# vimalabs/VIMA

Hardware: NVIDIA H100
Metric: policy steps/sec (batched action decode) (higher is better)
Workload: dtype f16 hi*hi + e4m3 cross terms (2 tensor pass-equivalents), f16 3-term in attention, fp32 accumulate/softmax/LN

## Files before the change

vima_b200/csrc/api.cu:

```cuda
#include <cstdarg>
#include <cstddef>
#include <cstdio>
#include <cstring>
#include <cstdlib>

#include "../../include/vima_b200.h"
#include "gemm_wide.cuh"
#include "kernels.h"

using namespace vima;
static_assert(VIMA_KV_PAGE_TOKENS == KV_PAGE_TOKENS, "page size of the C ABI and of the kernels");

struct vima_ctx {
  int device;
  int sm_count;
  int max_smem_optin;
  long long launches;
  char err[512];
  void* encode_tiled;
  int attn_tc;
  int attn_tail;
  int epi_prefetch;
  int attn_bias_tc;
  int gemm_wide;
};

struct DeviceGuard {
  int prev = -1;
  bool armed = false;
  cudaError_t enter(int dev) {
    cudaError_t e = cudaGetDevice(&prev);
    if (e != cudaSuccess) return e;
    if (prev == dev) return cudaSuccess;
    armed = true;
    return cudaSetDevice(dev);
  }
  ~DeviceGuard() {
    if (armed) cudaSetDevice(prev);
  }
};

static int fail(vima_ctx* c, int code, const char* fmt, ...) {
  if (c) {
    va_list ap;
    va_start(ap, fmt);
    vsnprintf(c->err, sizeof(c->err), fmt, ap);
    va_end(ap);
  }
  return code;
}
static int cuda_fail(vima_ctx* c, cudaError_t e, const char* what) {
  return fail(c, VIMA_E_CUDA, "%s: %s", what, cudaGetErrorString(e));
}
#define CHECK_CTX(c)                  \
  if (!(c)) return VIMA_E_INVALID;    \
  DeviceGuard dev_guard_;             \
  {                                   \
// ... 10 lines not shown
                what, sz, min_size, sizeof(D), VIMA_B200_ABI_VERSION);
  memset(out, 0, sizeof(D));
  memcpy(out, in, sz);
  return VIMA_OK;
}
#define LAUNCHED(c, expr, name)                          \
  {                                                      \
    cudaError_t e_ = (expr);                             \
    if (e_ != cudaSuccess) return cuda_fail((c), e_, name); \
    (c)->launches++;                                     \
    return VIMA_OK;                                      \
  }

extern "C" {

int vima_abi_version(void) { return VIMA_B200_ABI_VERSION; }

int vima_set_option(vima_ctx* c, const char* key, const char* value) {
  if (!c) return VIMA_E_INVALID;
  if (!key || !value) return fail(c, VIMA_E_INVALID, "set_option: null key or value");
  if (!strcmp(key, "attn")) {
    if (!strcmp(value, "tc")) { c->attn_tc = 1; return VIMA_OK; }
    if (!strcmp(value, "mma")) { c->attn_tc = 0; return VIMA_OK; }
  } else if (!strcmp(key, "attn_tail")) {
    if (!strcmp(value, "kernel")) { c->attn_tail = 1; return VIMA_OK; }
    if (!strcmp(value, "off")) { c->attn_tail = 0; return VIMA_OK; }
  } else if (!strcmp(key, "attn_bias")) {
    if (!strcmp(value, "auto")) { c->attn_bias_tc = 0; return VIMA_OK; }
    if (!strcmp(value, "tc")) { c->attn_bias_tc = 1; return VIMA_OK; }
  } else if (!strcmp(key, "epi_prefetch")) {
    if (!strcmp(value, "0") || !strcmp(value, "1")) { c->epi_prefetch = value[0] == '1'; return VIMA_OK; }
  } else if (!strcmp(key, "gemm_wide")) {
    if (!strcmp(value, "0") || !strcmp(value, "1")) { c->gemm_wide = value[0] == '1'; return VIMA_OK; }
  }
  return fail(c, VIMA_E_INVALID, "set_option: unknown option %s=%s", key, value);
}

int vima_create(vima_ctx** out, int device) {
  if (!out) return VIMA_E_INVALID;
  *out = nullptr;
  int n = 0;
  if (cudaGetDeviceCount(&n) != cudaSuccess || device < 0 || device >= n) return VIMA_E_CUDA;
  cudaDeviceProp prop;
  if (cudaGetDeviceProperties(&prop, device) != cudaSuccess) return VIMA_E_CUDA;
  if (prop.major != 9 || prop.minor != 0) return VIMA_E_UNSUPPORTED;
  vima_ctx* c = new vima_ctx();
  memset(c, 0, sizeof(*c));
  c->device = device;
  c->sm_count = prop.multiProcessorCount;
  c->max_smem_optin = (int)prop.sharedMemPerBlockOptin;
  DeviceGuard guard;
  if (guard.enter(device) != cudaSuccess) { delete c; return VIMA_E_CUDA; }
  cudaFree(0);
  cudaDriverEntryPointQueryResult q;
  void* fn = nullptr;
  if (cudaGetDriverEntryPoint("cuTensorMapEncodeTiled", &fn, cudaEnableDefault, &q) != cudaSuccess || fn == nullptr) {
    delete c;
    return VIMA_E_CUDA;
  }
  c->encode_tiled = fn;
  c->attn_tc = 1; c->attn_tail = 1; c->epi_prefetch = 0; c->attn_bias_tc = 0; c->gemm_wide = 1;
  if (const char* e = getenv("VIMA_B200_ATTN")) vima_set_option(c, "attn", e);
  if (const char* e = getenv("VIMA_B200_ATTN_TAIL")) vima_set_option(c, "attn_tail", e);
  if (const char* e = getenv("VIMA_B200_EPI_PREFETCH")) vima_set_option(c, "epi_prefetch", e);
  if (const char* e = getenv("VIMA_B200_ATTN_BIAS")) vima_set_option(c, "attn_bias", e);
  if (const char* e = getenv("VIMA_B200_GEMM_WIDE")) vima_set_option(c, "gemm_wide", e);
  c->err[0] = 0;
  *out = c;
  return VIMA_OK;
}

void vima_destroy(vima_ctx* c) { delete c; }
const char* vima_last_error(vima_ctx* c) { return c ? c->err : "null context"; }
int vima_sm_count(vima_ctx* c) { return c ? c->sm_count : 0; }
int vima_sizeof_gemm_desc(void) { return (int)sizeof(vima_gemm_desc); }
int vima_sizeof_norm_desc(void) { return (int)sizeof(vima_norm_desc); }
int vima_sizeof_attn_desc(void) { return (int)sizeof(vima_attn_desc); }
int vima_sizeof_f32_gemm_group(void) { return (int)sizeof(vima_f32_gemm_group); }
int64_t vima_launch_count(vima_ctx* c) { return c ? c->launches : 0; }

int vima_split_f32(vima_ctx* c, const float* x, int64_t rows, int cols, int ldx, void* hi, void* lo, int ld16, int pad_cols, float scale,
                   int dtype, void* stream) {
  CHECK_CTX(c);
  if (!x || !hi || pad_cols < cols || pad_cols > ld16) return fail(c, VIMA_E_INVALID, "split_f32: bad arguments");
  LAUNCHED(c, launch_split(x, rows, cols, ldx, (unsigned short*)hi, (unsigned short*)lo, ld16, pad_cols, scale, dtype, (cudaStream_t)stream),
           "split_f32");
}

int vima_pack_weight(vima_ctx* c, const float* w, int n, int k, int transposed, int ldw, void* hi, void* lo, int ld16, float scale, int dtype,
                     void* stream) {
  CHECK_CTX(c);
  if (!w || !hi || ld16 < k || (ld16 & 7)) return fail(c, VIMA_E_INVALID, "pack_weight: ld16 must be >= k and a multiple of 8");
  LAUNCHED(c, launch_pack_weight(w, n, k, transposed, ldw, (unsigned short*)hi, (unsigned short*)lo, ld16, scale, dtype, (cudaStream_t)stream),
           "pack_weight");
}

int vima_pack_weight_f8(vima_ctx* c, const float* w, int n, int k, int transposed, int ldw, void* hi8, void* lo8, int ld8, float scale, void* stream) {
  CHECK_CTX(c);
  if (!w || !hi8 || !lo8 || ld8 < k || (ld8 & 15)) return fail(c, VIMA_E_INVALID, "pack_weight_f8: ld8 must be >= k and a multiple of 16");
// ... 11 lines not shown
  const int step = glu ? 64 : 32;
  int best = step, best_pad = 1 << 30;
  for (int bn = step; bn <= GEMM_MAX_BN; bn += step) {
    const int padded = ((N + bn - 1) / bn) * bn;
    if (padded < best_pad || (padded == best_pad && bn > best)) { best = bn; best_pad = padded; }
  }
  return best;
}
int vima_glu_block_n(int n_out) { return choose_block_n(2 * n_out, 1); }
int vima_gemm_stats_parts(int N, int glu, int block_n) {
  const int bn = block_n > 0 ? block_n : choose_block_n(N, glu);
  return 2 * ((N + bn - 1) / bn);
}

int vima_row_stats_finalize(vima_ctx* c, const float* partial, int64_t rows, int parts, int cols, float eps, int rms, float* stats, void* stream) {
  CHECK_CTX(c);
  if (!partial || !stats || rows < 0 || parts <= 0 || cols <= 0 || ((uintptr_t)partial & 7) || ((uintptr_t)stats & 7))
    return fail(c, VIMA_E_INVALID, "row_stats_finalize: bad arguments");
  LAUNCHED(c, launch_row_stats_finalize(partial, rows, parts, cols, eps, rms, stats, (cudaStream_t)stream), "row_stats_finalize");
}

static int make_tmap_f8(vima_ctx* c, CUtensorMap* tm, const void* base, int rows, int cols, int ld, int box_rows) {
  CUresult r = encode_tmap_2d(c->encode_tiled, tm, CU_TENSOR_MAP_DATA_TYPE_UINT8, base, (uint64_t)rows, (uint64_t)cols, (uint64_t)ld, GEMM_BK,
                              (uint32_t)box_rows, CU_TENSOR_MAP_SWIZZLE_64B, CU_TENSOR_MAP_L2_PROMOTION_L2_256B);
  if (r != CUDA_SUCCESS) return fail(c, VIMA_E_CUDA, "cuTensorMapEncodeTiled(fp8) failed (%d): rows %d cols %d ld %d box %d", (int)r, rows, cols, ld, box_rows);
  return VIMA_OK;
}

static int make_tmap(vima_ctx* c, CUtensorMap* tm, const void* base, int dtype, int rows, int cols, int ld, int box_rows) {
  const CUtensorMapDataType dt = dtype == DT_BF16 ? CU_TENSOR_MAP_DATA_TYPE_BFLOAT16 : CU_TENSOR_MAP_DATA_TYPE_FLOAT16;
  CUresult r = encode_tmap_2d(c->encode_tiled, tm, dt, base, (uint64_t)rows, (uint64_t)cols, (uint64_t)ld * 2, GEMM_BK, (uint32_t)box_rows,
                              CU_TENSOR_MAP_SWIZZLE_128B, CU_TENSOR_MAP_L2_PROMOTION_L2_256B);
  if (r != CUDA_SUCCESS) return fail(c, VIMA_E_CUDA, "cuTensorMapEncodeTiled failed (%d): rows %d cols %d ld %d box %d", (int)r, rows, cols, ld, box_rows);
  return VIMA_OK;
}

int vima_gemm(vima_ctx* c, const vima_gemm_desc* d_in, void* stream) {
  CHECK_CTX(c);
  vima_gemm_desc d_local;
  if (int rc_ = load_desc(c, d_in, &d_local, VIMA_GEMM_DESC_V4_SIZE, "gemm")) return rc_;
  const vima_gemm_desc* d = &d_local;
  if (!d->a_hi || !d->b_hi) return fail(c, VIMA_E_INVALID, "gemm: null operand");
  if (d->M <= 0 || d->N <= 0 || d->K <= 0) return fail(c, VIMA_E_INVALID, "gemm: empty problem");
  if ((d->lda & 7) || (d->ldb & 7) || ((uintptr_t)d->a_hi & 15) || ((uintptr_t)d->b_hi & 15))
    return fail(c, VIMA_E_INVALID, "gemm: operands need 16-byte aligned bases and ld %% 8 == 0 (lda %d ldb %d)", d->lda, d->ldb);
  if ((d->a_lo == nullptr) != (d->b_lo == nullptr)) return fail(c, VIMA_E_INVALID, "gemm: a_lo and b_lo must both be set or both be null");
  const bool f8 = d->a_lo8 || d->a_hi8 || d->b_hi8 || d->b_lo8;
  if (f8) {
    if (!(d->a_lo8 && d->a_hi8 && d->b_hi8 && d->b_lo8) || d->a_lo || d->dtype != DT_F16)
      return fail(c, VIMA_E_INVALID, "gemm: f16f8 mode needs all four e4m3 operands, fp16 hi operands and no 16-bit lo operands");
    if ((d->lda8 & 15) || (d->ldb8 & 15) || ((uintptr_t)d->a_lo8 & 15) || ((uintptr_t)d->a_hi8 & 15) || ((uintptr_t)d->b_hi8 & 15) ||
        ((uintptr_t)d->b_lo8 & 15) || d->lda8 < d->K || d->ldb8 < d->K)
      return fail(c, VIMA_E_INVALID, "gemm: e4m3 operands need 16-byte aligned bases and ld %% 16 == 0");
  }
  if ((d->out_lo8 == nullptr) != (d->out_hi8 == nullptr) || (d->out_lo8 && (!d->out_hi || d->dtype != DT_F16 || (d->ld_o8 & 3))))
    return fail(c, VIMA_E_INVALID, "gemm: out_lo8/out_hi8 come together, with an fp16 out_hi, ld_o8 %% 4 == 0");
  if (d->lda < d->K || d->ldb < d->K) return fail(c, VIMA_E_INVALID, "gemm: leading dimension smaller than K");
  int bn = d->block_n > 0 ? d->block_n : choose_block_n(d->N, d->glu);
  if (bn > GEMM_MAX_BN || (bn % (d->glu ? 64 : 32))) return fail(c, VIMA_E_INVALID, "gemm: bad block_n %d (multiple of 32, 64 with GLU, <= %d)", bn, GEMM_MAX_BN);
  if (d->glu && (d->N % bn)) return fail(c, VIMA_E_INVALID, "gemm: GLU needs N %% block_n == 0");
  {
    const int n_out = d->glu ? d->N / 2 : d->N;
    const bool bad = (n_out & 3) || (d->out_f32 && ((d->ld_o32 & 3) || ((uintptr_t)d->out_f32 & 15))) ||
                     (d->out_hi && ((d->ld_o16 & 3) || ((uintptr_t)d->out_hi & 7) || (d->out_lo && ((uintptr_t)d->out_lo & 7)))) ||
                     (d->mul && ((d->ld_mul & 3) || ((uintptr_t)d->mul & 15))) || (d->residual && ((d->ld_res & 3) || ((uintptr_t)d->residual & 15)));
    if (bad) return fail(c, VIMA_E_INVALID, "gemm: epilogue tensors need N %% 4 == 0, ld %% 4 == 0 and 16-byte (fp32) / 8-byte (16-bit) aligned bases");
// ... 22 lines not shown
  l.split = split; l.block_n = bn;
  const bool wide = c->gemm_wide && split == 2 && bn == 128 && d->N % GEMM_WIDE_BN == 0 && gemm_wide_has_epilogue(l) &&
                    gemm_wide_smem_bytes() <= (size_t)c->max_smem_optin;
  const int tile_n = wide ? GEMM_WIDE_BN : bn;
  int rc;
  const int tiles_m_ = (d->M + GEMM_BM - 1) / GEMM_BM, tiles_n_ = (d->N + tile_n - 1) / tile_n;
  if ((rc = make_tmap(c, &p.tm_a_hi, d->a_hi, d->dtype, d->M, d->K, d->lda, GEMM_BM))) return rc;
  if ((rc = make_tmap(c, &p.tm_b_hi, d->b_hi, d->dtype, d->N, d->K, d->ldb, tile_n))) return rc;
  if (split == 1) {
    if ((rc = make_tmap(c, &p.tm_a_lo, d->a_lo, d->dtype, d->M, d->K, d->lda, GEMM_BM))) return rc;
    if ((rc = make_tmap(c, &p.tm_b_lo, d->b_lo, d->dtype, d->N, d->K, d->ldb, bn))) return rc;
  } else if (split == 2) {
    if ((rc = make_tmap_f8(c, &p.tm_a_lo, d->a_lo8, d->M, d->K, d->lda8, GEMM_BM))) return rc;
    if ((rc = make_tmap_f8(c, &p.tm_a_hi8, d->a_hi8, d->M, d->K, d->lda8, GEMM_BM))) return rc;
    if ((rc = make_tmap_f8(c, &p.tm_b_hi8, d->b_hi8, d->N, d->K, d->ldb8, tile_n))) return rc;
    if ((rc = make_tmap_f8(c, &p.tm_b_lo, d->b_lo8, d->N, d->K, d->ldb8, tile_n))) return rc;
  }
  p.M = d->M; p.N = d->N; p.K = d->K;
  p.dtype = d->dtype;
  p.glu = d->glu;
  p.epi_prefetch = c->epi_prefetch;
  p.act = d->act;
  p.acc_scale = d->acc_scale == 0.f ? 1.f : d->acc_scale;
  p.bias = d->bias;
  p.mul = d->mul; p.ld_mul = d->ld_mul;
  p.residual = d->residual; p.ld_res = d->ld_res;
  p.out_f32 = d->out_f32; p.ld_o32 = d->ld_o32;
  p.out_hi = (unsigned short*)d->out_hi; p.out_lo = (unsigned short*)d->out_lo; p.ld_o16 = d->ld_o16;
  p.out_lo8 = (unsigned char*)d->out_lo8; p.out_hi8 = (unsigned char*)d->out_hi8; p.ld_o8 = d->ld_o8;
  p.row_stats = d->row_stats; p.ln_c1 = d->ln_c1; p.ln_cols = d->ln_cols;
  p.res_stats = d->res_stats; p.res_gamma = d->res_gamma; p.res_beta = d->res_beta;
  p.stats_out = d->stats_out; p.stats_parts = d->stats_parts;

  const int tiles = tiles_m_ * tiles_n_;
  const int grid = tiles < c->sm_count ? tiles : c->sm_count;
  if (wide) LAUNCHED(c, launch_gemm_wide(p, l, grid, gemm_wide_smem_bytes(), c->max_smem_optin, (cudaStream_t)stream), "gemm_wide_kernel");
  const size_t stage = (size_t)(GEMM_A_TILE_BYTES + bn * 128) * (split ? 2 : 1);
  const size_t fixed = gemm_smem_bytes(bn, split, 0);
  int n_stages = (int)(((size_t)c->max_smem_optin - fixed) / stage);
  if (n_stages > GEMM_MAX_STAGES) n_stages = GEMM_MAX_STAGES;
  if (n_stages < 2) return fail(c, VIMA_E_UNSUPPORTED, "gemm: not enough shared memory for 2 stages");
  p.n_stages = n_stages;
  const size_t smem = gemm_smem_bytes(bn, split, n_stages);
  auto launch = d->dtype == DT_BF16 ? (split ? launch_gemm_tc<DT_BF16, 1> : launch_gemm_tc<DT_BF16, 0>)
                                    : (split == 2 ? launch_gemm_tc<DT_F16, 2> : split ? launch_gemm_tc<DT_F16, 1> : launch_gemm_tc<DT_F16, 0>);
  LAUNCHED(c, launch(p, l, grid, smem, c->max_smem_optin, (cudaStream_t)stream), "gemm_tc_kernel");
}

int vima_gemm_f32_grouped(vima_ctx* c, const vima_f32_gemm_group* groups_dev, int n_groups, int M, int max_n, int act, void* stream) {
  CHECK_CTX(c);
  static_assert(sizeof(vima_f32_gemm_group) == sizeof(SimtGemmGroup), "group layout");
  if (!groups_dev) return fail(c, VIMA_E_INVALID, "gemm_f32_grouped: null groups");
  LAUNCHED(c, launch_simt_gemm_grouped(reinterpret_cast<const SimtGemmGroup*>(groups_dev), n_groups, M, max_n, act, (cudaStream_t)stream),
           "simt_gemm");
}

int vima_gemm_f32_grouped_host(vima_ctx* c, const vima_f32_gemm_group* groups_host, int n_groups, int M, int max_n, int act, void* stream) {
  CHECK_CTX(c);
  if (!groups_host || n_groups < 0) return fail(c, VIMA_E_INVALID, "gemm_f32_grouped_host: null groups");
  if (M < 0) return fail(c, VIMA_E_INVALID, "gemm_f32_grouped_host: M = %d < 0", M);
  for (int i = 0; i < n_groups; ++i)
    if (groups_host[i].n > max_n)
      return fail(c, VIMA_E_INVALID, "gemm_f32_grouped_host: group %d has n = %d columns, more than max_n = %d", i, groups_host[i].n, max_n);
  cudaError_t e = launch_simt_gemm_grouped_host(reinterpret_cast<const SimtGemmGroup*>(groups_host), n_groups, M, max_n, act, (cudaStream_t)stream);
  if (e != cudaSuccess) return cuda_fail(c, e, "simt_gemm");
  c->launches += (n_groups + SIMT_MAX_HOST_GROUPS - 1) / SIMT_MAX_HOST_GROUPS;
// ... 341 lines not shown
```

vima_b200/csrc/common.cuh:

```cuda
#pragma once
#include <cuda.h>
#include <cuda_bf16.h>
#include <cuda_fp16.h>
#include <cuda_runtime.h>
#include <stdint.h>
#include <stdio.h>

#ifndef VIMA_WAIT_CYCLES
#define VIMA_WAIT_CYCLES (3000000000ll)
#endif

namespace vima {

enum : int { DT_F16 = 0, DT_BF16 = 1 };
enum : int { ACT_NONE = 0, ACT_RELU = 1, ACT_QUICKGELU = 2, ACT_GELU = 3, ACT_GELU_TANH = 4 };

__device__ __forceinline__ uint32_t smem_u32(const void* p) { return (uint32_t)__cvta_generic_to_shared(p); }

template <int DT>
struct Op16;
template <>
struct Op16<DT_F16> {
  using T = __half;
  static __device__ __forceinline__ unsigned short bits(float x) { return __half_as_ushort(__float2half_rn(x)); }
// ... 105 lines not shown
__device__ __forceinline__ void mbar_arrive(uint64_t* bar) {
  asm volatile("mbarrier.arrive.shared::cta.b64 _, [%0];" ::"r"(smem_u32(bar)) : "memory");
}
__device__ __forceinline__ bool mbar_try_wait(uint64_t* bar, uint32_t parity) {
  uint32_t ok;
  asm volatile(
      "{\n\t.reg .pred p;\n\t"
      "mbarrier.try_wait.parity.shared::cta.b64 p, [%1], %2;\n\t"
      "selp.u32 %0, 1, 0, p;\n\t}"
      : "=r"(ok)
      : "r"(smem_u32(bar)), "r"(parity)
      : "memory");
  return ok != 0;
}
__device__ __forceinline__ void mbar_wait(uint64_t* bar, uint32_t parity) {
  if (mbar_try_wait(bar, parity)) return;
  const long long t0 = clock64();
  uint32_t spins = 0;
  while (!mbar_try_wait(bar, parity)) {
    if ((++spins & 1023u) == 0u && clock64() - t0 > VIMA_WAIT_CYCLES) __trap();
  }
}

__device__ __forceinline__ void tma_prefetch_desc(const void* tmap) {
  asm volatile("prefetch.tensormap [%0];" ::"l"(tmap) : "memory");
}
__device__ __forceinline__ void tma_load_2d(void* smem_dst, const void* tmap, uint64_t* bar, int c0, int c1) {
  asm volatile(
      "cp.async.bulk.tensor.2d.shared::cluster.global.mbarrier::complete_tx::bytes [%0], [%1, {%3, %4}], [%2];" ::"r"(
          smem_u32(smem_dst)),
      "l"(tmap), "r"(smem_u32(bar)), "r"(c0), "r"(c1)
      : "memory");
}

__device__ __forceinline__ uint64_t wgmma_desc_sw128(uint32_t smem_addr) {
  return (uint64_t)((smem_addr >> 4) & 0x3FFF) | (1ull << 16) | ((uint64_t)(1024 >> 4) << 32) | (1ull << 62);
}
__device__ __forceinline__ uint64_t wgmma_desc_sw64(uint32_t smem_addr) {
  return (uint64_t)((smem_addr >> 4) & 0x3FFF) | (1ull << 16) | ((uint64_t)(512 >> 4) << 32) | (2ull << 62);
}
__device__ __forceinline__ void wgmma_fence() { asm volatile("wgmma.fence.sync.aligned;" ::: "memory"); }
__device__ __forceinline__ void wgmma_commit() { asm volatile("wgmma.commit_group.sync.aligned;" ::: "memory"); }
template <int N>
__device__ __forceinline__ void wgmma_wait() { asm volatile("wgmma.wait_group.sync.aligned %0;" ::"n"(N) : "memory"); }
template <int N>
__device__ __forceinline__ void wgmma_fence_acc(float (&d)[N]) {
#pragma unroll
  for (int i = 0; i < N; ++i) asm volatile("" : "+f"(d[i])::"memory");
}

#define VIMA_ACC8(d, o)                                                                                                  \
  "+f"(d[(o) + 0]), "+f"(d[(o) + 1]), "+f"(d[(o) + 2]), "+f"(d[(o) + 3]), "+f"(d[(o) + 4]), "+f"(d[(o) + 5]), "+f"(d[(o) + 6]), \
      "+f"(d[(o) + 7])
#define VIMA_ACC16(d) VIMA_ACC8(d, 0), VIMA_ACC8(d, 8)
#define VIMA_ACC32(d) VIMA_ACC16(d), VIMA_ACC8(d, 16), VIMA_ACC8(d, 24)
#define VIMA_ACC48(d) VIMA_ACC32(d), VIMA_ACC8(d, 32), VIMA_ACC8(d, 40)
#define VIMA_ACC64(d) VIMA_ACC48(d), VIMA_ACC8(d, 48), VIMA_ACC8(d, 56)
#define VIMA_R16 "{%0, %1, %2, %3, %4, %5, %6, %7, %8, %9, %10, %11, %12, %13, %14, %15}"
#define VIMA_R32 \
  "{%0, %1, %2, %3, %4, %5, %6, %7, %8, %9, %10, %11, %12, %13, %14, %15, %16, %17, %18, %19, %20, %21, %22, %23, %24, %25, %26, %27, %28, %29, %30, %31}"
#define VIMA_R48 \
  "{%0, %1, %2, %3, %4, %5, %6, %7, %8, %9, %10, %11, %12, %13, %14, %15, %16, %17, %18, %19, %20, %21, %22, %23, %24, %25, %26, %27, %28, %29, %30, %31, %32, %33, %34, %35, %36, %37, %38, %39, %40, %41, %42, %43, %44, %45, %46, %47}"
#define VIMA_R64 \
  "{%0, %1, %2, %3, %4, %5, %6, %7, %8, %9, %10, %11, %12, %13, %14, %15, %16, %17, %18, %19, %20, %21, %22, %23, %24, %25, %26, %27, %28, %29, %30, %31, %32, %33, %34, %35, %36, %37, %38, %39, %40, %41, %42, %43, %44, %45, %46, %47, %48, %49, %50, %51, %52, %53, %54, %55, %56, %57, %58, %59, %60, %61, %62, %63}"

#define VIMA_WGMMA_K16(N, R, ACC, IA, IB, IP)                                                                                      \
// ... 81 lines not shown
```

vima_b200/csrc/gemm_tc.cuh:

```cuda
#pragma once
#include "common.cuh"

namespace vima {

constexpr int GEMM_BM = 128;
constexpr int GEMM_BK = 64;
constexpr int GEMM_A_TILE_BYTES = GEMM_BM * 128;
constexpr int GEMM_CONSUMERS = 256;
constexpr int GEMM_THREADS = GEMM_CONSUMERS + 128;
constexpr int GEMM_PRODUCER_REGS = 40;
constexpr int GEMM_CONSUMER_REGS = 232;
constexpr int GEMM_MAX_BN = 128;
constexpr int GEMM_MAX_STAGES = 8;
constexpr int GEMM_STAGING_BYTES = 8 * 16 * 16 * 4;

struct alignas(64) GemmParams {
  CUtensorMap tm_a_hi, tm_a_lo, tm_b_hi, tm_b_lo;
  CUtensorMap tm_a_hi8, tm_b_hi8;
  int M, N, K;
  int n_stages;
  int dtype;
  int epi_prefetch;
  int glu;
  int act;
  float acc_scale;
  const float* bias;
  const float* mul;
  int ld_mul;
  const float* residual;
  int ld_res;
  float* out_f32;
  int ld_o32;
  unsigned short* out_hi;
  unsigned short* out_lo;
  int ld_o16;
  unsigned char* out_lo8;
  unsigned char* out_hi8;
  int ld_o8;
  const float* row_stats;
  const float* ln_c1;
  int ln_cols;
  const float* res_stats;
  const float* res_gamma;
  const float* res_beta;
  float* stats_out;
  int stats_parts;
};

template <bool GENERIC_, int ACT_, bool GLU_, bool MUL_, bool RES_, bool O32_, bool O16_, int DT_, bool LNA_ = false, bool LNR_ = false,
          bool STATS_ = false>
struct EpiCfg {
  static constexpr bool GENERIC = GENERIC_;
  static constexpr int ACT = ACT_;
  static constexpr bool GLU = GLU_, MUL = MUL_, RES = RES_, O32 = O32_, O16 = O16_;
  static constexpr int DT = DT_;
  static constexpr bool LNA = LNA_;
  static constexpr bool LNR = LNR_;
  static constexpr bool STATS = STATS_;
};

constexpr int GEMM_COLVEC_PLANES = 4;

template <int ACT>
__device__ __forceinline__ float act_ct(float x) {
  if constexpr (ACT == ACT_RELU) return fmaxf(x, 0.f);
  else if constexpr (ACT == ACT_QUICKGELU) return quick_gelu(x);
  else if constexpr (ACT == ACT_GELU) return gelu_erf(x);
  else if constexpr (ACT == ACT_GELU_TANH) return gelu_tanh(x);
  else return x;
}

template <int DT>
__device__ __forceinline__ void split4(const float4& y, uint2& hi, uint2& lo) { split4v<DT>(y, hi, lo); }

template <int BN>
__device__ __forceinline__ void acc_group16(const float (&acc)[BN / 2], int s, float (&v)[8]) {
#pragma unroll
  for (int t = 0; t < BN / 16; ++t)
    if (t == s) {
#pragma unroll
      for (int i = 0; i < 8; ++i) v[i] = acc[t * 8 + i];
    }
}

template <class E, int BN>
__device__ __forceinline__ void epilogue_tile(const GemmParams& p, const float (&acc)[BN / 2], const float* __restrict__ sb,
                                              float* __restrict__ st, int lane, int row_base, int tn, int bn_out, int n_out) {
  const bool glu = E::GENERIC ? (p.glu != 0) : E::GLU;
  const bool has_mul = E::GENERIC ? (p.mul != nullptr) : E::MUL;
  const bool has_res = E::GENERIC ? (p.residual != nullptr) : E::RES;
  const bool o32 = E::GENERIC ? (p.out_f32 != nullptr) : E::O32;
  const bool o16 = E::GENERIC ? (p.out_hi != nullptr) : E::O16;
  const bool lna = E::GENERIC ? (p.row_stats != nullptr) : E::LNA;
  const bool lnr = E::GENERIC ? (p.res_stats != nullptr) : E::LNR;
  const bool stats = E::GENERIC ? (p.stats_out != nullptr) : E::STATS;
  const float scale = p.acc_scale;
  const int sub = lane >> 2;
  const int kc = lane & 3;
  const float* sc1 = sb + 256;
  const float* sgam = sb + 512;
  const float* sbet = sb + 768;
  float a_mean[2] = {0.f, 0.f}, a_rstd[2] = {1.f, 1.f};
  if (lna) {
#pragma unroll
    for (int h = 0; h < 2; ++h) {
      const int row = row_base + sub + 8 * h;
      if (row < p.M) {
        const float2 ms = __ldg(reinterpret_cast<const float2*>(p.row_stats) + row);
        a_mean[h] = ms.x; a_rstd[h] = ms.y;
      }
    }
  }
  const bool ln_gate = lna && p.ln_cols == 1;
  float r_mean[2], r_rstd[2], st1[2][2], st2[2][2];
#pragma unroll
  for (int it = 0; it < 2; ++it) {
    r_mean[it] = 0.f; r_rstd[it] = 1.f;
    st1[0][it] = st1[1][it] = st2[0][it] = st2[1][it] = 0.f;
    if (lnr) {
      const int row = row_base + it * 8 + sub;
      if (row < p.M) {
        const float2 ms = __ldg(reinterpret_cast<const float2*>(p.res_stats) + row);
        r_mean[it] = ms.x; r_rstd[it] = ms.y;
      }
    }
  }
  auto load_mr = [&](int j, float4 (&mm_)[2], float4 (&rr_)[2]) {
    const int col = tn * bn_out + j + kc * 4;
    const bool col_ok = col < n_out;
#pragma unroll
    for (int it = 0; it < 2; ++it) {
      const int row = row_base + it * 8 + sub;
      const bool ok = col_ok && row < p.M;
      if (has_mul) mm_[it] = ok ? __ldg(reinterpret_cast<const float4*>(p.mul + (size_t)row * p.ld_mul + col)) : make_float4(1.f, 1.f, 1.f, 1.f);
      if (has_res) rr_[it] = ok ? __ldg(reinterpret_cast<const float4*>(p.residual + (size_t)row * p.ld_res + col)) : make_float4(0.f, 0.f, 0.f, 0.f);
    }
  };
  float4 mm[2], rr[2], mm_n[2], rr_n[2];
  load_mr(0, mm, rr);
  const int wsw = (sub >> 1) & 3;
#pragma unroll
  for (int s = 0; s < BN / 16; ++s) {
    const int j = s * 16;
    if (j < bn_out) {
      const int col = tn * bn_out + j + kc * 4;
      const bool col_ok = col < n_out;
      if (j + 16 < bn_out) load_mr(j + 16, mm_n, rr_n);
      float v[8], g[8], x[8];
#pragma unroll
      for (int i = 0; i < 8; ++i) v[i] = acc[s * 8 + i];
      if (glu) acc_group16<BN>(acc, s + bn_out / 16, g);
#pragma unroll
      for (int i = 0; i < 8; ++i) {
        const int c = j + 8 * (i >> 2) + 2 * kc + (i & 1);
        const int h = (i >> 1) & 1;
        float a;
        if (lna) a = fmaf(fmaf(-a_mean[h], sc1[c], v[i] * scale), a_rstd[h], sb[c]);
        else a = fmaf(v[i], scale, sb[c]);
        if (glu) {
          float gt;
          if (ln_gate) gt = fmaf(fmaf(-a_mean[h], sc1[bn_out + c], g[i] * scale), a_rstd[h], sb[bn_out + c]);
          else gt = fmaf(g[i], scale, sb[bn_out + c]);
          a = E::GENERIC ? apply_act(p.act, a) : act_ct<E::ACT>(a);
          x[i] = a * gt;
        } else {
          x[i] = E::GENERIC ? apply_act(p.act, a) : act_ct<E::ACT>(a);
        }
      }
#pragma unroll
      for (int q = 0; q < 2; ++q)
#pragma unroll
        for (int h = 0; h < 2; ++h) {
          const int r = sub + 8 * h;
          const int ch = (2 * q + (kc >> 1)) ^ wsw;
          *reinterpret_cast<float2*>(st + r * 16 + ch * 4 + (2 * kc & 3)) = make_float2(x[4 * q + 2 * h], x[4 * q + 2 * h + 1]);
        }
      __syncwarp();
      float4 y[2];
#pragma unroll
      for (int it = 0; it < 2; ++it) {
        const int r = it * 8 + sub;
        y[it] = *reinterpret_cast<const float4*>(st + r * 16 + ((kc ^ ((r >> 1) & 3)) << 2));
      }
      const int half = (j >> 5) & 1;
#pragma unroll
      for (int it = 0; it < 2; ++it) {
        const int row = row_base + it * 8 + sub;
        if (!(col_ok && row < p.M)) continue;
        float4 o = y[it];
        if (has_mul) { o.x *= mm[it].x; o.y *= mm[it].y; o.z *= mm[it].z; o.w *= mm[it].w; }
        if (has_res) {
          float4 r = rr[it];
          if (lnr) {
            const float4 gm = *reinterpret_cast<const float4*>(sgam + j + kc * 4);
            const float4 bt = *reinterpret_cast<const float4*>(sbet + j + kc * 4);
            const float m_ = r_mean[it], s_ = r_rstd[it];
            r.x = fmaf((r.x - m_) * s_, gm.x, bt.x); r.y = fmaf((r.y - m_) * s_, gm.y, bt.y);
            r.z = fmaf((r.z - m_) * s_, gm.z, bt.z); r.w = fmaf((r.w - m_) * s_, gm.w, bt.w);
          }
          o.x += r.x; o.y += r.y; o.z += r.z; o.w += r.w;
        }
        if (stats) {
          st1[half][it] += (o.x + o.y) + (o.z + o.w);
          st2[half][it] += fmaf(o.x, o.x, o.y * o.y) + fmaf(o.z, o.z, o.w * o.w);
        }
        if (o32) *reinterpret_cast<float4*>(p.out_f32 + (size_t)row * p.ld_o32 + col) = o;
        if (o16) {
          if (p.out_lo8) {
            uint2 h16;
            uint32_t l8, h8;
            split4_f8(o, F8_ACT_LO_SCALE, F8_ACT_HI_SCALE, h16, l8, h8);
            *reinterpret_cast<uint2*>(p.out_hi + (size_t)row * p.ld_o16 + col) = h16;
            *reinterpret_cast<uint32_t*>(p.out_lo8 + (size_t)row * p.ld_o8 + col) = l8;
            *reinterpret_cast<uint32_t*>(p.out_hi8 + (size_t)row * p.ld_o8 + col) = h8;
          } else {
            uint2 hi, lo;
            if (E::GENERIC) {
              if (p.dtype == DT_F16) split4<DT_F16>(o, hi, lo); else split4<DT_BF16>(o, hi, lo);
            } else {
              split4<E::DT>(o, hi, lo);
            }
            *reinterpret_cast<uint2*>(p.out_hi + (size_t)row * p.ld_o16 + col) = hi;
            if (p.out_lo) *reinterpret_cast<uint2*>(p.out_lo + (size_t)row * p.ld_o16 + col) = lo;
          }
        }
      }
      __syncwarp();
#pragma unroll
      for (int it = 0; it < 2; ++it) {
        if (has_mul) mm[it] = mm_n[it];
        if (has_res) rr[it] = rr_n[it];
      }
    }
  }
  if (stats) {
#pragma unroll
    for (int hf = 0; hf < 2; ++hf)
#pragma unroll
      for (int it = 0; it < 2; ++it) {
        float s1 = st1[hf][it], s2 = st2[hf][it];
        s1 += __shfl_xor_sync(0xffffffffu, s1, 1); s2 += __shfl_xor_sync(0xffffffffu, s2, 1);
        s1 += __shfl_xor_sync(0xffffffffu, s1, 2); s2 += __shfl_xor_sync(0xffffffffu, s2, 2);
        const int row = row_base + it * 8 + sub;
        if (kc == 0 && row < p.M) reinterpret_cast<float2*>(p.stats_out)[(size_t)row * p.stats_parts + tn * 2 + hf] = make_float2(s1, s2);
      }
  }
}

template <class E, int SPLIT, int BN>
__global__ void __launch_bounds__(GEMM_THREADS, 1) gemm_tc_kernel(const __grid_constant__ GemmParams p) {
  static_assert(SPLIT >= 0 && SPLIT <= 2 && BN % 32 == 0 && BN <= GEMM_MAX_BN, "gemm_tc_kernel: bad SPLIT / BN");
  extern __shared__ __align__(1024) uint8_t smem_raw[];
  uint8_t* smem = (uint8_t*)(((uintptr_t)smem_raw + 1023) & ~(uintptr_t)1023);
  constexpr int b_tile_bytes = BN * 128;
  constexpr int n_parts = SPLIT ? 2 : 1;
  constexpr int stage_bytes = (GEMM_A_TILE_BYTES + b_tile_bytes) * n_parts;
  uint8_t* stages = smem;
  float* staging = (float*)(smem + (size_t)p.n_stages * stage_bytes);
// ... 169 lines not shown
```

vima_b200/csrc/gemm_wide.cuh:

```cuda
#pragma once
#include "gemm_tc_variants.cuh"

namespace vima {

constexpr int GEMM_WIDE_BN = 256;
constexpr int GEMM_WIDE_A16 = GEMM_BM * GEMM_BK * 2;
constexpr int GEMM_WIDE_A8 = GEMM_BM * GEMM_BK;
constexpr int GEMM_WIDE_B16 = GEMM_WIDE_BN * GEMM_BK * 2;
constexpr int GEMM_WIDE_B8 = GEMM_WIDE_BN * GEMM_BK;
constexpr int GEMM_WIDE_STAGE_BYTES = GEMM_WIDE_A16 + GEMM_WIDE_B16;
static_assert(GEMM_WIDE_STAGE_BYTES == 2 * GEMM_WIDE_A8 + 2 * GEMM_WIDE_B8, "the fp16 and the e4m3 half-blocks fill a slot each");
constexpr int GEMM_WIDE_STAGES = 4;

#define VIMA_R128                                                                                                                  \
  "{%0, %1, %2, %3, %4, %5, %6, %7, %8, %9, %10, %11, %12, %13, %14, %15, %16, %17, %18, %19, %20, %21, %22, %23, %24, %25, %26, "  \
  "%27, %28, %29, %30, %31, %32, %33, %34, %35, %36, %37, %38, %39, %40, %41, %42, %43, %44, %45, %46, %47, %48, %49, %50, %51, "   \
  "%52, %53, %54, %55, %56, %57, %58, %59, %60, %61, %62, %63, %64, %65, %66, %67, %68, %69, %70, %71, %72, %73, %74, %75, %76, "   \
  "%77, %78, %79, %80, %81, %82, %83, %84, %85, %86, %87, %88, %89, %90, %91, %92, %93, %94, %95, %96, %97, %98, %99, %100, %101, " \
  "%102, %103, %104, %105, %106, %107, %108, %109, %110, %111, %112, %113, %114, %115, %116, %117, %118, %119, %120, %121, %122, "  \
  "%123, %124, %125, %126, %127}"
#define VIMA_U8(d, o)                                                                                                           \
  "+r"(d[(o) + 0]), "+r"(d[(o) + 1]), "+r"(d[(o) + 2]), "+r"(d[(o) + 3]), "+r"(d[(o) + 4]), "+r"(d[(o) + 5]), "+r"(d[(o) + 6]), \
      "+r"(d[(o) + 7])
#define VIMA_U64(d) VIMA_U8(d, 0), VIMA_U8(d, 8), VIMA_U8(d, 16), VIMA_U8(d, 24), VIMA_U8(d, 32), VIMA_U8(d, 40), VIMA_U8(d, 48), VIMA_U8(d, 56)

__device__ __forceinline__ void wgmma_m64n256k16_f16(float (&d0)[64], float (&d1)[64], uint64_t da, uint64_t db) {
  asm volatile("wgmma.mma_async.sync.aligned.m64n256k16.f32.f16.f16 " VIMA_R128 ", %128, %129, 1, 1, 1, 0, 0;"
               : VIMA_ACC64(d0), VIMA_ACC64(d1)
               : "l"(da), "l"(db));
}
__device__ __forceinline__ void wgmma_m64n256k32_e4m3_f16(uint32_t (&d)[64], uint64_t da, uint64_t db) {
  asm volatile("wgmma.mma_async.sync.aligned.m64n256k32.f16.e4m3.e4m3 " VIMA_R64 ", %64, %65, 1, 1, 1;"
               : VIMA_U64(d)
               : "l"(da), "l"(db));
}
#undef VIMA_U64
#undef VIMA_U8
#undef VIMA_R128

template <int N>
__device__ __forceinline__ void wgmma_fence_acc(uint32_t (&d)[N]) {
#pragma unroll
  for (int i = 0; i < N; ++i) asm volatile("" : "+r"(d[i])::"memory");
}

template <class E>
__global__ void __launch_bounds__(GEMM_THREADS, 1) gemm_wide_kernel(const __grid_constant__ GemmParams p) {
  extern __shared__ __align__(1024) uint8_t smem_raw[];
  uint8_t* smem = (uint8_t*)(((uintptr_t)smem_raw + 1023) & ~(uintptr_t)1023);
  constexpr int BN = GEMM_WIDE_BN;
  constexpr int off_b16 = GEMM_WIDE_A16;
  constexpr int off_a_hi8 = GEMM_WIDE_A8, off_b_hi8 = 2 * GEMM_WIDE_A8, off_b_lo8 = off_b_hi8 + GEMM_WIDE_B8;
  uint8_t* stages = smem;
  float* staging = (float*)(smem + GEMM_WIDE_STAGES * GEMM_WIDE_STAGE_BYTES);
  float* sbias = staging + GEMM_STAGING_BYTES / 4;
  uint64_t* bars = (uint64_t*)(sbias + 2 * GEMM_COLVEC_PLANES * 256);
  uint64_t* full_bar = bars;
  uint64_t* empty_bar = bars + GEMM_WIDE_STAGES;

  const int warp = threadIdx.x >> 5;
  const int lane = threadIdx.x & 31;

  const int tiles_m = (p.M + GEMM_BM - 1) / GEMM_BM;
  const int tiles_n = (p.N + BN - 1) / BN;
  const int num_kb = (p.K + GEMM_BK - 1) / GEMM_BK;
  const int num_tiles = tiles_m * tiles_n;

  if (threadIdx.x == GEMM_CONSUMERS) {
    tma_prefetch_desc(&p.tm_a_hi);
    tma_prefetch_desc(&p.tm_b_hi);
    tma_prefetch_desc(&p.tm_a_lo);
    tma_prefetch_desc(&p.tm_b_lo);
    tma_prefetch_desc(&p.tm_a_hi8);
    tma_prefetch_desc(&p.tm_b_hi8);
    for (int s = 0; s < GEMM_WIDE_STAGES; ++s) {
      mbar_init(&full_bar[s], 1);
      mbar_init(&empty_bar[s], GEMM_CONSUMERS / 32);
    }
    fence_barrier_init();
  }
  __syncthreads();

  if (warp >= GEMM_CONSUMERS / 32) {
    setmaxnreg_dec<GEMM_PRODUCER_REGS>();
    if (threadIdx.x == GEMM_CONSUMERS) {
      int pair = 0;
      uint32_t phase = 0;
      for (int tile = blockIdx.x; tile < num_tiles; tile += gridDim.x) {
        const int m0 = (tile / tiles_n) * GEMM_BM;
        const int n0 = (tile % tiles_n) * BN;
        for (int kb = 0; kb < num_kb; ++kb) {
          const int k0 = kb * GEMM_BK;
          const int s16 = 2 * pair, s8 = 2 * pair + 1;
          uint8_t* st16 = stages + (size_t)s16 * GEMM_WIDE_STAGE_BYTES;
          uint8_t* st8 = stages + (size_t)s8 * GEMM_WIDE_STAGE_BYTES;
          mbar_wait(&empty_bar[s16], phase ^ 1);
          mbar_arrive_expect_tx(&full_bar[s16], (uint32_t)GEMM_WIDE_STAGE_BYTES);
          tma_load_2d(st16, &p.tm_a_hi, &full_bar[s16], k0, m0);
          tma_load_2d(st16 + off_b16, &p.tm_b_hi, &full_bar[s16], k0, n0);
          mbar_wait(&empty_bar[s8], phase ^ 1);
          mbar_arrive_expect_tx(&full_bar[s8], (uint32_t)GEMM_WIDE_STAGE_BYTES);
          tma_load_2d(st8, &p.tm_a_lo, &full_bar[s8], k0, m0);
          tma_load_2d(st8 + off_a_hi8, &p.tm_a_hi8, &full_bar[s8], k0, m0);
          tma_load_2d(st8 + off_b_hi8, &p.tm_b_hi8, &full_bar[s8], k0, n0);
          tma_load_2d(st8 + off_b_lo8, &p.tm_b_lo, &full_bar[s8], k0, n0);
          pair ^= 1;
          if (pair == 0) phase ^= 1;
// ... 50 lines not shown
      for (int k = 0; k < GEMM_BK / 16; ++k)
        wgmma_m64n256k16_f16(acc0, acc1, da_hi + 2 * k, db_hi + 2 * k);
      wgmma_commit();
      wgmma_wait<1>();
      if (prev_stage >= 0 && lane == 0) mbar_arrive(&empty_bar[prev_stage]);
      mbar_wait(&full_bar[s8], phase);
      const uint32_t b8 = smem_u32(stages + (size_t)s8 * GEMM_WIDE_STAGE_BYTES);
      const uint64_t da_lo8 = wgmma_desc_sw64(b8 + a8_off), db_hi8 = wgmma_desc_sw64(b8 + off_b_hi8);
      const uint64_t da_hi8 = wgmma_desc_sw64(b8 + off_a_hi8 + a8_off), db_lo8 = wgmma_desc_sw64(b8 + off_b_lo8);
      wgmma_fence();
#pragma unroll
      for (int k = 0; k < GEMM_BK / 32; ++k) {
        wgmma_m64n256k32_e4m3_f16(acc8, da_lo8 + 2 * k, db_hi8 + 2 * k);
        wgmma_m64n256k32_e4m3_f16(acc8, da_hi8 + 2 * k, db_lo8 + 2 * k);
      }
      wgmma_commit();
      wgmma_wait<1>();
      if (lane == 0) mbar_arrive(&empty_bar[s16]);
      prev_stage = s8;
      pair ^= 1;
      if (pair == 0) phase ^= 1;
    }
    wgmma_wait<0>();
    wgmma_fence_acc(acc0);
    wgmma_fence_acc(acc1);
    wgmma_fence_acc(acc8);
#pragma unroll
    for (int r = 0; r < 32; ++r) {
      const float2 lo = __half22float2(*reinterpret_cast<const __half2*>(&acc8[r]));
      const float2 hi = __half22float2(*reinterpret_cast<const __half2*>(&acc8[32 + r]));
      acc0[2 * r] += lo.x; acc0[2 * r + 1] += lo.y;
      acc1[2 * r] += hi.x; acc1[2 * r + 1] += hi.y;
    }
    if (prev_stage >= 0 && lane == 0) mbar_arrive(&empty_bar[prev_stage]);
    float* sb = sbias + ab * (GEMM_COLVEC_PLANES * 256);
    for (int c = et; c < BN; c += GEMM_CONSUMERS) {
      sb[c] = (p.bias != nullptr && n0 + c < p.N) ? __ldg(p.bias + n0 + c) : 0.f;
      if (E::GENERIC ? (p.row_stats != nullptr) : E::LNA) sb[256 + c] = (n0 + c < p.N) ? __ldg(p.ln_c1 + n0 + c) : 0.f;
      if (E::GENERIC ? (p.res_stats != nullptr) : E::LNR) {
        const int oc = tn * bn_out + c;
        const bool okc = c < bn_out && oc < n_out;
        sb[512 + c] = okc ? __ldg(p.res_gamma + oc) : 0.f;
        sb[768 + c] = okc ? __ldg(p.res_beta + oc) : 0.f;
      }
    }
    named_bar_sync(1, GEMM_CONSUMERS);
    const int row_base = m0 + wg * 64 + (warp & 3) * 16;
    epilogue_tile<E, 128>(p, acc0, sb, st, lane, row_base, 2 * tn, bn_out / 2, n_out);
    epilogue_tile<E, 128>(p, acc1, sb + 128, st, lane, row_base, 2 * tn + 1, bn_out / 2, n_out);
    ab ^= 1;
  }
}

constexpr size_t gemm_wide_smem_bytes() {
  return 1024  + (size_t)GEMM_WIDE_STAGES * GEMM_WIDE_STAGE_BYTES + GEMM_STAGING_BYTES + 2 * GEMM_COLVEC_PLANES * 256 * 4 +
         2 * GEMM_WIDE_STAGES * 8 + 16;
}

bool gemm_wide_has_epilogue(const GemmLaunch& l);
cudaError_t launch_gemm_wide(const GemmParams& p, const GemmLaunch& l, int grid, size_t smem, int max_smem, cudaStream_t stream);

}
```

Measured before the change: 1625.

## Stage wide-GEMM epilogue outputs in smem and write them with TMA bulk stores

The wide GEMM epilogue can now write its fp32/fp16/e4m3 outputs into per-warp shared-memory staging buffers carved from the tile's last pipeline slot. It then issues cp.async.bulk tensor stores instead of per-thread global stores, replacing scattered 16-byte writes with bulk 16x16 tile stores. The pipeline slot is held until the bulk reads finish, which delays its release to the producer and adds proxy fences and wait_group stalls. It is enabled by default and falls back to direct stores when pointers or pitches are not 16-byte aligned.

```diff
diff --git a/vima_b200/csrc/api.cu b/vima_b200/csrc/api.cu
--- a/vima_b200/csrc/api.cu
+++ b/vima_b200/csrc/api.cu
@@ -23,6 +23,7 @@
   int epi_prefetch;
   int attn_bias_tc;
   int gemm_wide;
+  int gemm_epi_tma;
 };
 
 struct DeviceGuard {
@@ -99,6 +100,8 @@
     if (!strcmp(value, "0") || !strcmp(value, "1")) { c->epi_prefetch = value[0] == '1'; return VIMA_OK; }
   } else if (!strcmp(key, "gemm_wide")) {
     if (!strcmp(value, "0") || !strcmp(value, "1")) { c->gemm_wide = value[0] == '1'; return VIMA_OK; }
+  } else if (!strcmp(key, "gemm_epi_tma")) {
+    if (!strcmp(value, "0") || !strcmp(value, "1")) { c->gemm_epi_tma = value[0] == '1'; return VIMA_OK; }
   }
   return fail(c, VIMA_E_INVALID, "set_option: unknown option %s=%s", key, value);
 }
@@ -126,12 +129,13 @@
     return VIMA_E_CUDA;
   }
   c->encode_tiled = fn;
-  c->attn_tc = 1; c->attn_tail = 1; c->epi_prefetch = 0; c->attn_bias_tc = 0; c->gemm_wide = 1;
+  c->attn_tc = 1; c->attn_tail = 1; c->epi_prefetch = 0; c->attn_bias_tc = 0; c->gemm_wide = 1; c->gemm_epi_tma = 1;
   if (const char* e = getenv("VIMA_B200_ATTN")) vima_set_option(c, "attn", e);
   if (const char* e = getenv("VIMA_B200_ATTN_TAIL")) vima_set_option(c, "attn_tail", e);
   if (const char* e = getenv("VIMA_B200_EPI_PREFETCH")) vima_set_option(c, "epi_prefetch", e);
   if (const char* e = getenv("VIMA_B200_ATTN_BIAS")) vima_set_option(c, "attn_bias", e);
   if (const char* e = getenv("VIMA_B200_GEMM_WIDE")) vima_set_option(c, "gemm_wide", e);
+  if (const char* e = getenv("VIMA_B200_GEMM_EPI_TMA")) vima_set_option(c, "gemm_epi_tma", e);
   c->err[0] = 0;
   *out = c;
   return VIMA_OK;
@@ -209,6 +213,13 @@
   CUresult r = encode_tmap_2d(c->encode_tiled, tm, dt, base, (uint64_t)rows, (uint64_t)cols, (uint64_t)ld * 2, GEMM_BK, (uint32_t)box_rows,
                               CU_TENSOR_MAP_SWIZZLE_128B, CU_TENSOR_MAP_L2_PROMOTION_L2_256B);
   if (r != CUDA_SUCCESS) return fail(c, VIMA_E_CUDA, "cuTensorMapEncodeTiled failed (%d): rows %d cols %d ld %d box %d", (int)r, rows, cols, ld, box_rows);
+  return VIMA_OK;
+}
+
+static int make_tmap_out(vima_ctx* c, CUtensorMap* tm, CUtensorMapDataType dt, const void* base, int rows, int cols, size_t ld_bytes) {
+  CUresult r = encode_tmap_2d(c->encode_tiled, tm, dt, base, (uint64_t)rows, (uint64_t)cols, (uint64_t)ld_bytes, 16, 16,
+                              CU_TENSOR_MAP_SWIZZLE_NONE, CU_TENSOR_MAP_L2_PROMOTION_NONE);
+  if (r != CUDA_SUCCESS) return fail(c, VIMA_E_CUDA, "cuTensorMapEncodeTiled(output) failed (%d): rows %d cols %d ld %zu B", (int)r, rows, cols, ld_bytes);
   return VIMA_OK;
 }
 
@@ -297,6 +308,24 @@
   p.res_stats = d->res_stats; p.res_gamma = d->res_gamma; p.res_beta = d->res_beta;
   p.stats_out = d->stats_out; p.stats_parts = d->stats_parts;
 
+  if (wide && c->gemm_epi_tma) {
+    const int n_out = d->glu ? d->N / 2 : d->N;
+    const auto a16 = [](const void* q) { return ((uintptr_t)q & 15) == 0; };
+    const auto pitch = [n_out](int ld, int elem) { return ld >= n_out && ((size_t)ld * elem) % 16 == 0; };
+    const bool ok = (!d->out_f32 || (a16(d->out_f32) && pitch(d->ld_o32, 4))) &&
+                    (!d->out_hi || (a16(d->out_hi) && (!d->out_lo || a16(d->out_lo)) && pitch(d->ld_o16, 2))) &&
+                    (!d->out_lo8 || (a16(d->out_lo8) && a16(d->out_hi8) && pitch(d->ld_o8, 1)));
+    if (ok) {
+      if (d->out_f32 && (rc = make_tmap_out(c, &p.tm_o32, CU_TENSOR_MAP_DATA_TYPE_FLOAT32, d->out_f32, d->M, n_out, (size_t)d->ld_o32 * 4))) return rc;
+      if (d->out_hi && (rc = make_tmap_out(c, &p.tm_o16, CU_TENSOR_MAP_DATA_TYPE_UINT16, d->out_hi, d->M, n_out, (size_t)d->ld_o16 * 2))) return rc;
+      if (d->out_lo && (rc = make_tmap_out(c, &p.tm_o16_lo, CU_TENSOR_MAP_DATA_TYPE_UINT16, d->out_lo, d->M, n_out, (size_t)d->ld_o16 * 2))) return rc;
+      if (d->out_lo8) {
+        if ((rc = make_tmap_out(c, &p.tm_o8_lo, CU_TENSOR_MAP_DATA_TYPE_UINT8, d->out_lo8, d->M, n_out, (size_t)d->ld_o8))) return rc;
+        if ((rc = make_tmap_out(c, &p.tm_o8_hi, CU_TENSOR_MAP_DATA_TYPE_UINT8, d->out_hi8, d->M, n_out, (size_t)d->ld_o8))) return rc;
+      }
+      p.epi_tma = 1;
+    }
+  }
   const int tiles = tiles_m_ * tiles_n_;
   const int grid = tiles < c->sm_count ? tiles : c->sm_count;
   if (wide) LAUNCHED(c, launch_gemm_wide(p, l, grid, gemm_wide_smem_bytes(), c->max_smem_optin, (cudaStream_t)stream), "gemm_wide_kernel");
diff --git a/vima_b200/csrc/common.cuh b/vima_b200/csrc/common.cuh
--- a/vima_b200/csrc/common.cuh
+++ b/vima_b200/csrc/common.cuh
@@ -161,6 +161,14 @@
       "l"(tmap), "r"(smem_u32(bar)), "r"(c0), "r"(c1)
       : "memory");
 }
+__device__ __forceinline__ void tma_store_2d(const void* tmap, const void* smem_src, int c0, int c1) {
+  asm volatile("cp.async.bulk.tensor.2d.global.shared::cta.bulk_group [%0, {%2, %3}], [%1];" ::"l"(tmap), "r"(smem_u32(smem_src)),
+               "r"(c0), "r"(c1)
+               : "memory");
+}
+__device__ __forceinline__ void bulk_commit() { asm volatile("cp.async.bulk.commit_group;" ::: "memory"); }
+template <int N>
+__device__ __forceinline__ void bulk_wait_read() { asm volatile("cp.async.bulk.wait_group.read %0;" ::"n"(N) : "memory"); }
 
 __device__ __forceinline__ uint64_t wgmma_desc_sw128(uint32_t smem_addr) {
   return (uint64_t)((smem_addr >> 4) & 0x3FFF) | (1ull << 16) | ((uint64_t)(1024 >> 4) << 32) | (1ull << 62);
diff --git a/vima_b200/csrc/gemm_tc.cuh b/vima_b200/csrc/gemm_tc.cuh
--- a/vima_b200/csrc/gemm_tc.cuh
+++ b/vima_b200/csrc/gemm_tc.cuh
@@ -17,6 +17,8 @@
 struct alignas(64) GemmParams {
   CUtensorMap tm_a_hi, tm_a_lo, tm_b_hi, tm_b_lo;
   CUtensorMap tm_a_hi8, tm_b_hi8;
+  CUtensorMap tm_o32, tm_o16, tm_o16_lo, tm_o8_lo, tm_o8_hi;
+  int epi_tma;
   int M, N, K;
   int n_stages;
   int dtype;
@@ -83,9 +85,17 @@
     }
 }
 
-template <class E, int BN>
+constexpr int EPI_TMA_BUF_BYTES = 2048;
+constexpr int EPI_TMA_BUFS = 3;
+struct EpiStaging {
+  uint8_t* base;
+  int buf;
+};
+
+template <class E, int BN, bool TMA = false>
 __device__ __forceinline__ void epilogue_tile(const GemmParams& p, const float (&acc)[BN / 2], const float* __restrict__ sb,
-                                              float* __restrict__ st, int lane, int row_base, int tn, int bn_out, int n_out) {
+                                              float* __restrict__ st, int lane, int row_base, int tn, int bn_out, int n_out,
+                                              EpiStaging* stg = nullptr) {
   const bool glu = E::GENERIC ? (p.glu != 0) : E::GLU;
   const bool has_mul = E::GENERIC ? (p.mul != nullptr) : E::MUL;
   const bool has_res = E::GENERIC ? (p.residual != nullptr) : E::RES;
@@ -146,6 +156,7 @@
       const int col = tn * bn_out + j + kc * 4;
       const bool col_ok = col < n_out;
       if (j + 16 < bn_out) load_mr(j + 16, mm_n, rr_n);
+      if (TMA && lane == 0) bulk_wait_read<EPI_TMA_BUFS - 1>();
       float v[8], g[8], x[8];
 #pragma unroll
       for (int i = 0; i < 8; ++i) v[i] = acc[s * 8 + i];
@@ -183,10 +194,12 @@
         y[it] = *reinterpret_cast<const float4*>(st + r * 16 + ((kc ^ ((r >> 1) & 3)) << 2));
       }
       const int half = (j >> 5) & 1;
+      uint8_t* sbuf = TMA ? stg->base + stg->buf * EPI_TMA_BUF_BYTES : nullptr;
 #pragma unroll
       for (int it = 0; it < 2; ++it) {
         const int row = row_base + it * 8 + sub;
-        if (!(col_ok && row < p.M)) continue;
+        const bool ok = col_ok && row < p.M;
+        if (!TMA && !ok) continue;
         float4 o = y[it];
         if (has_mul) { o.x *= mm[it].x; o.y *= mm[it].y; o.z *= mm[it].z; o.w *= mm[it].w; }
         if (has_res) {
@@ -200,9 +213,29 @@
           }
           o.x += r.x; o.y += r.y; o.z += r.z; o.w += r.w;
         }
-        if (stats) {
+        if (stats && ok) {
           st1[half][it] += (o.x + o.y) + (o.z + o.w);
           st2[half][it] += fmaf(o.x, o.x, o.y * o.y) + fmaf(o.z, o.z, o.w * o.w);
+        }
+        if constexpr (TMA) {
+          const int r = it * 8 + sub;
+          if (o32) *reinterpret_cast<float4*>(sbuf + r * 64 + kc * 16) = o;
+          if (o16) {
+            if (p.out_lo8) {
+              uint2 h16;
+              uint32_t l8, h8;
+              split4_f8(o, F8_ACT_LO_SCALE, F8_ACT_HI_SCALE, h16, l8, h8);
+              *reinterpret_cast<uint2*>(sbuf + 1024 + r * 32 + kc * 8) = h16;
+              *reinterpret_cast<uint32_t*>(sbuf + 1536 + r * 16 + kc * 4) = l8;
+              *reinterpret_cast<uint32_t*>(sbuf + 1792 + r * 16 + kc * 4) = h8;
+            } else {
+              uint2 hi, lo;
+              split4<E::DT>(o, hi, lo);
+              *reinterpret_cast<uint2*>(sbuf + 1024 + r * 32 + kc * 8) = hi;
+              if (p.out_lo) *reinterpret_cast<uint2*>(sbuf + 1536 + r * 32 + kc * 8) = lo;
+            }
+          }
+          continue;
         }
         if (o32) *reinterpret_cast<float4*>(p.out_f32 + (size_t)row * p.ld_o32 + col) = o;
         if (o16) {
@@ -224,6 +257,27 @@
             if (p.out_lo) *reinterpret_cast<uint2*>(p.out_lo + (size_t)row * p.ld_o16 + col) = lo;
           }
         }
+      }
+      if constexpr (TMA) {
+        fence_proxy_async();
+        __syncwarp();
+        const int c0 = tn * bn_out + j;
+        if (lane == 0) {
+          if (row_base < p.M && c0 < n_out) {
+            if (o32) tma_store_2d(&p.tm_o32, sbuf, c0, row_base);
+            if (o16) {
+              tma_store_2d(&p.tm_o16, sbuf + 1024, c0, row_base);
+              if (p.out_lo8) {
+                tma_store_2d(&p.tm_o8_lo, sbuf + 1536, c0, row_base);
+                tma_store_2d(&p.tm_o8_hi, sbuf + 1792, c0, row_base);
+              } else if (p.out_lo) {
+                tma_store_2d(&p.tm_o16_lo, sbuf + 1536, c0, row_base);
+              }
+            }
+          }
+          bulk_commit();
+        }
+        stg->buf = stg->buf == EPI_TMA_BUFS - 1 ? 0 : stg->buf + 1;
       }
       __syncwarp();
 #pragma unroll
diff --git a/vima_b200/csrc/gemm_wide.cuh b/vima_b200/csrc/gemm_wide.cuh
--- a/vima_b200/csrc/gemm_wide.cuh
+++ b/vima_b200/csrc/gemm_wide.cuh
@@ -11,6 +11,8 @@
 constexpr int GEMM_WIDE_STAGE_BYTES = GEMM_WIDE_A16 + GEMM_WIDE_B16;
 static_assert(GEMM_WIDE_STAGE_BYTES == 2 * GEMM_WIDE_A8 + 2 * GEMM_WIDE_B8, "the fp16 and the e4m3 half-blocks fill a slot each");
 constexpr int GEMM_WIDE_STAGES = 4;
+static_assert(GEMM_CONSUMERS / 32 * EPI_TMA_BUFS * EPI_TMA_BUF_BYTES == GEMM_WIDE_STAGE_BYTES,
+              "the TMA-store epilogue stages every consumer warp's outputs in the tile's last slot");
 
 #define VIMA_R128                                                                                                                  \
   "{%0, %1, %2, %3, %4, %5, %6, %7, %8, %9, %10, %11, %12, %13, %14, %15, %16, %17, %18, %19, %20, %21, %22, %23, %24, %25, %26, "  \
@@ -73,6 +75,12 @@
     tma_prefetch_desc(&p.tm_b_lo);
     tma_prefetch_desc(&p.tm_a_hi8);
     tma_prefetch_desc(&p.tm_b_hi8);
+    if (p.epi_tma) {
+      if (p.out_f32) tma_prefetch_desc(&p.tm_o32);
+      if (p.out_hi) tma_prefetch_desc(&p.tm_o16);
+      if (p.out_lo) tma_prefetch_desc(&p.tm_o16_lo);
+      if (p.out_lo8) { tma_prefetch_desc(&p.tm_o8_lo); tma_prefetch_desc(&p.tm_o8_hi); }
+    }
     for (int s = 0; s < GEMM_WIDE_STAGES; ++s) {
       mbar_init(&full_bar[s], 1);
       mbar_init(&empty_bar[s], GEMM_CONSUMERS / 32);
@@ -189,7 +197,8 @@
       acc0[2 * r] += lo.x; acc0[2 * r + 1] += lo.y;
       acc1[2 * r] += hi.x; acc1[2 * r + 1] += hi.y;
     }
-    if (prev_stage >= 0 && lane == 0) mbar_arrive(&empty_bar[prev_stage]);
+    const bool epi_tma = p.epi_tma != 0;
+    if (!epi_tma && lane == 0) mbar_arrive(&empty_bar[prev_stage]);
     float* sb = sbias + ab * (GEMM_COLVEC_PLANES * 256);
     for (int c = et; c < BN; c += GEMM_CONSUMERS) {
       sb[c] = (p.bias != nullptr && n0 + c < p.N) ? __ldg(p.bias + n0 + c) : 0.f;
@@ -203,8 +212,18 @@
     }
     named_bar_sync(1, GEMM_CONSUMERS);
     const int row_base = m0 + wg * 64 + (warp & 3) * 16;
-    epilogue_tile<E, 128>(p, acc0, sb, st, lane, row_base, 2 * tn, bn_out / 2, n_out);
-    epilogue_tile<E, 128>(p, acc1, sb + 128, st, lane, row_base, 2 * tn + 1, bn_out / 2, n_out);
+    if (epi_tma) {
+      EpiStaging stg{stages + (size_t)prev_stage * GEMM_WIDE_STAGE_BYTES + warp * (EPI_TMA_BUFS * EPI_TMA_BUF_BYTES), 0};
+      epilogue_tile<E, 128, true>(p, acc0, sb, st, lane, row_base, 2 * tn, bn_out / 2, n_out, &stg);
+      epilogue_tile<E, 128, true>(p, acc1, sb + 128, st, lane, row_base, 2 * tn + 1, bn_out / 2, n_out, &stg);
+      if (lane == 0) {
+        bulk_wait_read<0>();
+        mbar_arrive(&empty_bar[prev_stage]);
+      }
+    } else {
+      epilogue_tile<E, 128>(p, acc0, sb, st, lane, row_base, 2 * tn, bn_out / 2, n_out);
+      epilogue_tile<E, 128>(p, acc1, sb + 128, st, lane, row_base, 2 * tn + 1, bn_out / 2, n_out);
+    }
     ab ^= 1;
   }
 }
```

New measurement: 1644 (median of 6 runs). 1.01x the previous value.
